# norabelrose/sparse-vae

Hardware: AMD Instinct MI355X
Metric: training tokens/sec + ELBO match vs CPU ref, 512-tok seq, 1/2/4/8 MI355X (higher is better)
Workload: dtype bf16; 1 GPU; c2: TransformerVAE 6L d512 heads 8 seq 512, batch 64/GPU, dense attention, dropout 0.1, fwd+bwd+allreduce+clip+RAdam; model=TransformerVAE-6L-d512, global_batch=64, seq_len=512, parallelism=dp1

## Files before the change

include/svae.h:

```cpp
#ifndef SVAE_H
#define SVAE_H
#include <stdint.h>
#ifdef __cplusplus
extern "C" {
#endif

typedef void* svae_stream_t;

enum svae_epi {
  SVAE_EPI_BF16 = 0,
  SVAE_EPI_F32 = 1,
  SVAE_EPI_F32_ACC = 2,
  SVAE_EPI_F32_ATOMIC = 3,
  SVAE_EPI_GELU = 4,
  SVAE_EPI_GELU_BWD = 5,
  SVAE_EPI_DROPOUT_RESID = 6,
  SVAE_EPI_ROTARY_BF16 = 7,
  SVAE_EPI_CE_STATS = 8,
  SVAE_EPI_CE_PROB = 9,
  SVAE_EPI_ROWSCALE_GATHER = 10
};

typedef struct svae_gemm_desc {
  const void* A;
// ... 15 lines not shown
  uint64_t seed;
  const float* rot_tab;
  int32_t rot_cols, rot_d, rot_seq;
  const int32_t* labels;
  float* label_logit;
  float* a_rowsum;
  const float* k_weight;
  const float* row_a;
  const float* row_b;
  const void* gather;
  int64_t ldg;
  float* delta;
  const float* delta_o32;
  int64_t ld_o32;
  int32_t delta_hd, delta_seq;
} svae_gemm_desc;

int svae_gemm(const svae_gemm_desc* d, svae_stream_t stream);

int svae_gemm_pair(const svae_gemm_desc* d0, const svae_gemm_desc* d1, svae_stream_t stream);

#define SVAE_GROUP_MAX 256
#define SVAE_GROUP_MAX_BLOCKS 1024
int64_t svae_gemm_group_table_bytes(int32_t n);
int svae_gemm_group(const svae_gemm_desc* d, int32_t n, int32_t max_blocks, void* table, void* table_host,
                    int64_t table_bytes, svae_stream_t stream);

int svae_resid_ln_fwd(const float* x, const void* y, int32_t y_dtype, int64_t ldy, float drop_p, uint64_t seed,
                      const float* zrows, int32_t zmod, const float* w, const float* b, float* xo, void* h, float* mean,
                      float* rstd, int32_t rows, int32_t D, svae_stream_t stream);
// ... 18 lines not shown
int svae_layernorm_bwd_multi(const void* const* dy, const float* x, const float* const* w, const float* mean,
                             const float* rstd, const float* dres, float* dx, float* const* part, int32_t nblk,
                             int32_t n, int32_t rows, int32_t D, svae_stream_t stream);

int svae_colsum(const void* in, int32_t in_dtype, int32_t rows, int32_t cols, int64_t ld, float* out,
                int32_t accumulate, svae_stream_t stream);

#define SVAE_COLSUM_MAX 8
typedef struct svae_colsum_seg {
  const float* in;
  float* out;
  int64_t ld;
  int32_t rows, cols;
} svae_colsum_seg;
int svae_colsum_multi(const svae_colsum_seg* segs, int32_t n, svae_stream_t stream);

typedef struct svae_attn_desc {
  const void* q; const void* k; const void* v; void* o;
  int64_t sq, sk, sv, so, bq, bk, bv, bo;
  const uint8_t* key_pad;
  float* lse;
  int32_t B, H, Lq, Lk, hd, causal;
  float scale;
  const void* dout; int64_t sdo, bdo;
  float* delta;
  float* dq;
  int64_t bdq;
  void* dk; void* dv;
  int64_t sdk, sdv, bdk, bdv;
  const float* rot_tab;
// ... 153 lines not shown
```

sparse-vae_amd/csrc/gemm.hip:

```cpp
#include "common.h"
#include "../../include/svae.h"
#include <stdlib.h>
#include <string.h>
#include <algorithm>
#include <vector>

using namespace svae;

namespace {

constexpr int BM = 128, BN = 128, BK = 64;
constexpr int TILE_BYTES = BM * BK * 2;

struct GP {
  const bf16* A; const bf16* B;
  long long lda, ldb, sA, sB;
  int M, N, K, splits, kchunk, tiles_n, tiles_m;
  void* C; long long ldc, sC;
  const float* bias;
  const float* resid; long long ldr;
  void* aux; long long ldaux;
  float alpha, drop_p;
  unsigned long long seed;
  const float* rot_tab; int rot_cols, rot_d, rot_seq;
  const int* labels; float* label_logit;
  float* a_rowsum;
  const float* k_weight;
  const float* row_a; const float* row_b;
  const bf16* gather; long long ldg;
  int epi;
  int tn2, tm2;
  int group;
  int total3;
  int relaxed;
  int dma_stagger;
  long long slab;
  float* delta; const float* delta_o32; long long ld_o32; int delta_hd, delta_seq;
};

__device__ __forceinline__ int kc_off(int row, int c) { return row * 128 + ((c ^ ((row >> 1) & 7)) << 4); }
__device__ __forceinline__ int mn_off(int k, int u) {
  const int s = (k & 3) | (((k >> 3) & 1) << 2);
  return k * 256 + ((u ^ (s << 2)) << 3);
}

template <bool TRANS>
__device__ __forceinline__ void load_tile(const bf16* __restrict__ g, long long ld, int row0, int nrows, int k0,
                                          int kend, u32x4 (&r)[4], int tid) {
  const bf16* base = TRANS ? g + (long long)k0 * ld + row0 : g + (long long)row0 * ld + k0;
  const __amdgpu_buffer_rsrc_t rsrc = __builtin_amdgcn_make_buffer_rsrc((void*)base, 0, 0x7FFFFFF0, 0x00020000);
#pragma unroll
  for (int i = 0; i < 4; ++i) {
// ... 491 lines not shown
            cs[row * 128 + cs_swz(row, col)] = p.alpha * acc[i][j][r];
          }
    }
    __syncthreads();
    epilogue_half<EPI>(p, cs, m0, n0, bn, h * 64, cofs, tid);
    __syncthreads();
  }
}

constexpr int G3_T = 256 * 64 * 2;
constexpr int G3_STAGE = 2 * G3_T;
constexpr int G3_EPI_BF16_DELTA = 65;
constexpr int G3_EPI_ACC_KW = 64;
constexpr int G3_EPI_F32_KW = 66;
constexpr int G3_EPI_SLAB = 67;

struct G3Src {
  int off[4];
};

__device__ __forceinline__ void g3_piece_k(int piece, int lane, int& r, int& c) {
  r = piece * 8 + (lane >> 3);
  c = (lane & 7) ^ ((r >> 1) & 7);
}
__device__ __forceinline__ void g3_piece_mn(int piece, int lane, int& kr, int& col) {
  const int half = piece >> 4;
  kr = (piece & 15) * 4 + (lane >> 4);
  const int sk = (kr & 3) | (((kr >> 3) & 1) << 2);
  col = half * 128 + (((lane & 15) ^ (sk << 1)) * 8);
}
// ... 481 lines not shown
#ifndef SVAE_KW_FORM
#define SVAE_KW_FORM 0
#endif
#ifndef SVAE_KW_PRE
#define SVAE_KW_PRE 1
#endif

template <int EPI>
constexpr int g3_epi_vmem_ops() {
  switch (EPI) {
    case SVAE_EPI_BF16:
    case G3_EPI_BF16_DELTA:
    case SVAE_EPI_ROTARY_BF16:
    case SVAE_EPI_CE_STATS:
    case SVAE_EPI_ROWSCALE_GATHER:
    case SVAE_EPI_GELU_BWD:
      return 8 * 2;
    case SVAE_EPI_CE_PROB:
      return 8 * 2 + 1;
    case SVAE_EPI_GELU:
      return 8 * 2 * 2;
    case SVAE_EPI_F32:
    case SVAE_EPI_F32_ACC:
    case SVAE_EPI_DROPOUT_RESID:
    case G3_EPI_ACC_KW:
    case G3_EPI_F32_KW:
    case G3_EPI_SLAB:
      return 8 * 4;
    default:
      return 0;
  }
}

template <bool AT, bool BT, int EPI>
__device__ __forceinline__ void gemm256_run(const GP& p, int blk, int nwg, bool remap = true) {
  static_assert(g3_epi_vmem_ops<EPI>() >= G3_EPI_STORES, "the relaxed first wait would not cover the prefetch DMA");
  constexpr bool IS_KW = EPI == G3_EPI_ACC_KW || EPI == G3_EPI_F32_KW;
  constexpr int KW_FORM = IS_KW ? SVAE_KW_FORM : 0;
  constexpr int KW_SLOT = KW_FORM == 2 ? 1024 : 256;
  constexpr int KW_BYTES = KW_FORM ? 2 * 8 * KW_SLOT : 0;
  constexpr int RING_OFF = KW_FORM == 3 ? KW_BYTES : 0;
  constexpr int KW_OFF = KW_FORM == 3 ? 0 : 2 * G3_STAGE + 2048 + 8192;
  __shared__ __attribute__((aligned(16))) char smem[2 * G3_STAGE + 2048 + 8192 + KW_BYTES];
  char* ring = smem + RING_OFF;
  float* sbias = (float*)(ring + 2 * G3_STAGE);
  int* slabel = (int*)(ring + 2 * G3_STAGE + 1024);
  float* sstat = (float*)(ring + 2 * G3_STAGE + 2048);
  const int tid = threadIdx.x, lane = tid & 63;
  const int wave = __builtin_amdgcn_readfirstlane(tid >> 6);
  const int wr = wave >> 2, wc = wave & 3;
  int bid = blk;
  if (remap && nwg >= 16) {
    const int q = nwg / 8, r = nwg % 8, xcd = bid % 8, idx = bid / 8;
    bid = (xcd < r ? xcd * (q + 1) : r * (q + 1) + (xcd - r) * q) + idx;
  }
  int t3 = bid;
  if (t3 >= p.total3) return;
  G3Tile T = g3_tile(p, t3);
// ... 19 lines not shown
  bool relaxed = false;
  int ntile = 0;
  (void)ntile;
  while (true) {
    G3_STAMP(0);
    const int t3n = t3 + nwg;
    const bool has_next = t3n < p.total3;
    float rsum[4] = {0.f, 0.f, 0.f, 0.f};
    f32x4 acc[8][4];
#pragma unroll
    for (int i = 0; i < 8; ++i)
#pragma unroll
      for (int j = 0; j < 4; ++j) acc[i][j] = (f32x4){0.f, 0.f, 0.f, 0.f};

    const bool next_dma = has_next && g3_tile(p, t3n).nk > 0;
    for (int kt = 0; kt < T.nk; ++kt, ++g) {
      if (kt == 0 && relaxed) asm volatile("s_waitcnt vmcnt(%0)" ::"n"(G3_EPI_STORES) : "memory");
      else asm volatile("s_waitcnt vmcnt(0)" ::: "memory");
      __builtin_amdgcn_s_barrier();
      const char* la = ring + (g & 1) * G3_STAGE;
      const char* lb = la + G3_T;
      char* nxt = ring + ((g + 1) & 1) * G3_STAGE;
      const bool do_rs = AT && p.a_rowsum && T.bn < 2;
      const int ks0 = p.tn2 >= 2 ? T.bn : 0, ks1 = p.tn2 >= 2 ? T.bn + 1 : 2;
      const bool kw_pre = IS_KW && KW_FORM == 0 && SVAE_KW_PRE && do_rs;
      float kw1 = 0.f;
      if (kw_pre) {
        const int kk = T.kbeg + kt * 64 + lane_id_fresh();
        const int off = kk < T.kend ? kk * 4 : 0x7FFFFFF0;
        const u32x4 kwr = buffer_rsrc(p.k_weight, 0x7FFFFFF0u);
        asm volatile("s_nop 4\n\tbuffer_load_dword %0, %1, %2, 0 offen" : "=&v"(kw1) : "v"(off), "s"(kwr) : "memory");
      }
      const bool late = (!IS_KW || KW_FORM > 0 || kw_pre) && p.dma_stagger && wr == 1 && kt + 1 < T.nk;
      if (kt + 1 < T.nk) {
        if (!late) g3_issue<AT, BT>(p, T.A, T.B, sa, sb, T.m0, T.n0, T.kbeg + (kt + 1) * 64, T.kend, nxt, wave);
        kw_issue(T.kbeg + (kt + 1) * 64, T.kend, (g + 1) & 1);
      } else if (next_dma) {
        const G3Tile TN = g3_tile(p, t3n);
// ... 50 lines not shown
#pragma unroll
      for (int j = 0; j < 2; ++j)
#pragma unroll
        for (int ks = 0; ks < 2; ++ks) b1[j][ks] = g3_bfrag<BT>(lb, wc * 64 + 32 + j * 16, ks, lane);
#pragma unroll
      for (int ks = 0; ks < 2; ++ks)
#pragma unroll
        for (int i = 0; i < 4; ++i)
#pragma unroll
          for (int j = 0; j < 2; ++j) acc[i][j] = mfma16(b0[j][ks], a0[i][ks], acc[i][j]);
      if (late) {
        __builtin_amdgcn_sched_barrier(0);
        g3_issue<AT, BT>(p, T.A, T.B, sa, sb, T.m0, T.n0, T.kbeg + (kt + 1) * 64, T.kend, nxt, wave);
        __builtin_amdgcn_sched_barrier(0);
      }
      if constexpr (!AT) {
#pragma unroll
        for (int i = 0; i < 4; ++i)
#pragma unroll
          for (int ks = 0; ks < 2; ++ks) a1[i][ks] = g3_afrag<AT>(la, wr * 128 + 64 + i * 16, ks, lane);
      }
#pragma unroll
      for (int ks = 0; ks < 2; ++ks)
#pragma unroll
        for (int i = 0; i < 4; ++i)
#pragma unroll
          for (int j = 0; j < 2; ++j) acc[i][2 + j] = mfma16(b1[j][ks], a0[i][ks], acc[i][2 + j]);
      if constexpr (AT) {
        if (kw_pre) asm volatile("s_waitcnt vmcnt(8)" : "+v"(kw1) :: "memory");
        if (do_rs) {
// ... 11 lines not shown
        for (int i = 0; i < 4; ++i)
#pragma unroll
          for (int j = 0; j < 2; ++j) acc[4 + i][2 + j] = mfma16(b1[j][ks], a1[i][ks], acc[4 + i][2 + j]);
#pragma unroll
      for (int ks = 0; ks < 2; ++ks)
#pragma unroll
        for (int i = 0; i < 4; ++i)
#pragma unroll
          for (int j = 0; j < 2; ++j) acc[4 + i][j] = mfma16(b0[j][ks], a1[i][ks], acc[4 + i][j]);
      if constexpr (AT) {
        if (do_rs) {
          if (wc == 2) rowsum2(a1[0], a1[1]);
          else if (wc == 3) rowsum2(a1[2], a1[3]);
        }
      }
    }
    G3_STAMP(1);
    if (tid < 256) {
      const int n = T.n0 + tid, m = T.m0 + tid;
      sbias[tid] = (p.bias && n < p.N) ? p.bias[n] : 0.f;
      if (EPI == SVAE_EPI_CE_STATS || EPI == SVAE_EPI_CE_PROB || EPI == SVAE_EPI_ROWSCALE_GATHER)
        slabel[tid] = m < p.M ? p.labels[m] : 0;
      if (EPI == SVAE_EPI_CE_PROB) sstat[1024 + tid] = (m < p.M && p.labels[m] != 0) ? p.row_a[m] : INFINITY;
      if (EPI == SVAE_EPI_ROWSCALE_GATHER) sstat[1024 + tid] = m < p.M ? p.row_a[m] : 0.f;
      if (EPI == SVAE_EPI_ROWSCALE_GATHER) sstat[1280 + tid] = m < p.M ? p.row_b[m] : 0.f;
    }
    asm volatile("s_waitcnt lgkmcnt(0)" ::: "memory");
    __builtin_amdgcn_s_barrier();
    if constexpr (AT) {
      if (p.a_rowsum && T.bn < 2) {
#pragma unroll
        for (int h = 0; h < 2; ++h) {
          const float t = sum_x16_x32(rsum[h]);
          const int m = T.m0 + wr * 128 + (2 * wc + h) * 16 + (lane & 15);
          if ((lane >> 4) == 0 && m < p.M) atomicAdd(p.a_rowsum + m, t);
        }
      }
    }
    if constexpr (EPI == SVAE_EPI_BF16 || EPI == SVAE_EPI_GELU || EPI == SVAE_EPI_CE_STATS ||
                  EPI == SVAE_EPI_ROTARY_BF16 || EPI == SVAE_EPI_CE_PROB)
      g3_reg_epilogue<EPI>(p, acc, sbias, slabel, sstat, T.m0, T.n0, T.bn, T.batch, T.split, wr, wc, tid, lane);
    else if constexpr (EPI == SVAE_EPI_ROWSCALE_GATHER)
      g3_rowscale_gather_epilogue(p, acc, slabel, sstat + 1024, sstat + 1280, T.m0, T.n0, wr, wc, lane);
    else if constexpr (EPI == SVAE_EPI_F32 || EPI == SVAE_EPI_F32_ACC || EPI == SVAE_EPI_DROPOUT_RESID ||
                       EPI == SVAE_EPI_GELU_BWD || EPI == G3_EPI_BF16_DELTA)
      g3_reg_epilogue_ld<EPI>(p, acc, sbias, T.m0, T.n0, T.batch, T.split, wr, wc, lane);
    else if constexpr (EPI == G3_EPI_ACC_KW)
      g3_reg_epilogue_ld<SVAE_EPI_F32_ACC>(p, acc, sbias, T.m0, T.n0, T.batch, T.split, wr, wc, lane);
    else if constexpr (EPI == G3_EPI_F32_KW || EPI == G3_EPI_SLAB)
      g3_reg_epilogue_ld<G3_EPI_SLAB>(p, acc, sbias, T.m0, T.n0, T.batch, T.split, wr, wc, lane);
    else
      static_assert(EPI == G3_EPI_SLAB, "no gemm256 epilogue for this EPI");
    relaxed = p.relaxed && T.m0 + 256 <= p.M && T.n0 + 256 <= p.N;
    G3_STAMP(2);
    ++ntile;
    if (!has_next) break;
    const bool prefetched = T.nk > 0;
// ... 167 lines not shown
__global__ __launch_bounds__(256) void slab_reduce_kernel(SlabRed r) { slab_reduce_range(r, blockIdx.x, gridDim.x); }
__global__ __launch_bounds__(256) void slab_reduce2_kernel(SlabRed r0, SlabRed r1, int nb0) {
  if ((int)blockIdx.x < nb0) slab_reduce_range(r0, blockIdx.x, nb0);
  else slab_reduce_range(r1, blockIdx.x - nb0, (int)gridDim.x - nb0);
}
struct alignas(16) SlabRedSlot {
  SlabRed r;
};
__global__ __launch_bounds__(256) void slab_reduce_list_kernel(const SlabRedSlot* __restrict__ list, int n) {
  for (int e = 0; e < n; ++e) {
    const SlabRed r = load_uniform(&list[e].r);
    slab_reduce_range(r, blockIdx.x, gridDim.x);
  }
}

}

static SlabRed slab_red(const svae_gemm_desc* d) {
  return SlabRed{(const float*)d->aux, (float*)d->C, d->M, d->N, (long long)d->ldc, d->splits};
}
static long long slab_blocks(const svae_gemm_desc* d) {
  return std::min(4096LL, ((long long)d->M * (d->N / 4) + 255) / 256);
}
static int launch_slab_reduce(const svae_gemm_desc* d, hipStream_t s) {
  hipLaunchKernelGGL(slab_reduce_kernel, dim3((unsigned)slab_blocks(d)), dim3(256), 0, s, slab_red(d));
  SVAE_LAUNCH_CHECK();
  return SVAE_OK;
}

static int validate_desc(const svae_gemm_desc* d) {
// ... 10 lines not shown
  if (d->epi == SVAE_EPI_CE_PROB && !d->aux) return SVAE_EINVAL;
  if (d->epi == SVAE_EPI_ROWSCALE_GATHER && (!d->row_b || !d->gather || d->ldg % 8 || ((uintptr_t)d->gather & 15)))
    return SVAE_EINVAL;
  if (d->k_weight && (!d->a_rowsum || !d->a_t || (d->splits != 1 && !(d->epi == SVAE_EPI_F32_ATOMIC && d->aux))))
    return SVAE_EINVAL;
  if (d->epi == SVAE_EPI_ROTARY_BF16 && (!d->rot_tab || d->rot_d <= 0 || d->rot_seq <= 0)) return SVAE_EINVAL;
  if ((d->epi == SVAE_EPI_GELU || d->epi == SVAE_EPI_GELU_BWD || d->epi == SVAE_EPI_CE_STATS) && !d->aux)
    return SVAE_EINVAL;
  if (d->epi == SVAE_EPI_DROPOUT_RESID && !d->resid) return SVAE_EINVAL;
  if ((d->epi == SVAE_EPI_DROPOUT_RESID || d->epi == SVAE_EPI_F32) && d->aux &&
      (d->batch != 1 || d->ldaux % 8 || ((uintptr_t)d->aux & 15)))
    return SVAE_EINVAL;
  if (d->epi == SVAE_EPI_CE_STATS && (!d->labels || !d->label_logit || d->splits != 1)) return SVAE_EINVAL;
  if (d->splits > 1 && d->epi != SVAE_EPI_F32_ATOMIC) return SVAE_EINVAL;
  if (d->a_rowsum && !d->a_t) return SVAE_EINVAL;
  if (d->N % 4 || d->ldc % 8 || ((uintptr_t)d->C & 15) || (d->resid && (d->ldr % 4 || ((uintptr_t)d->resid & 15))))
    return SVAE_EINVAL;
  if ((d->epi == SVAE_EPI_GELU || d->epi == SVAE_EPI_GELU_BWD) && (d->ldaux % 8 || ((uintptr_t)d->aux & 15)))
    return SVAE_EINVAL;
  if (d->epi == SVAE_EPI_ROTARY_BF16 && (d->rot_d % 4 || d->rot_cols % 4)) return SVAE_EINVAL;

  return SVAE_OK;
}

static void fill_gp(const svae_gemm_desc* d, GP& p) {
  p.A = (const bf16*)d->A; p.B = (const bf16*)d->B;
  p.lda = d->lda; p.ldb = d->ldb; p.sA = d->batch_stride_a; p.sB = d->batch_stride_b;
  p.M = d->M; p.N = d->N; p.K = d->K; p.splits = d->splits;
  int kchunk = (d->K + d->splits - 1) / d->splits;
  kchunk = (kchunk + BK - 1) / BK * BK;
// ... 3 lines not shown
  p.C = d->C; p.ldc = d->ldc; p.sC = d->batch_stride_c;
  p.bias = d->bias; p.resid = d->resid; p.ldr = d->ldr;
  p.aux = d->aux; p.ldaux = d->ldaux;
  p.alpha = d->alpha; p.drop_p = d->drop_p; p.seed = d->seed;
  p.rot_tab = d->rot_tab; p.rot_cols = d->rot_cols; p.rot_d = d->rot_d; p.rot_seq = d->rot_seq;
  p.labels = d->labels; p.label_logit = d->label_logit;
  p.a_rowsum = d->a_rowsum;
  p.k_weight = d->k_weight;
  p.row_a = d->row_a; p.row_b = d->row_b;
  p.gather = (const bf16*)d->gather; p.ldg = d->ldg;
  p.epi = d->epi;
  p.slab = 0;
  p.dma_stagger = 0;
  p.delta = d->delta; p.delta_o32 = d->delta_o32; p.ld_o32 = d->ld_o32;
  p.delta_hd = d->delta_hd; p.delta_seq = d->delta_seq;
}

__global__ __launch_bounds__(256) void gemm_delta_kernel(const bf16* __restrict__ C, long long ldc,
                                                         const float* __restrict__ o32, long long ldo, int M, int H,
                                                         int hd, int seq, float* __restrict__ delta) {
  const int gw = blockIdx.x * 4 + (threadIdx.x >> 6), lane = threadIdx.x & 63;
  if (gw >= M * H) return;
  const int m = gw / H, h = gw - m * H;
  float s = 0.f;
  for (int c = lane * 4; c < hd; c += 256) {
    const bf16x4 a = *(const bf16x4*)(C + (long long)m * ldc + h * hd + c);
    const f32x4 o = *(const f32x4*)(o32 + (long long)m * ldo + h * hd + c);
#pragma unroll
    for (int e = 0; e < 4; ++e) s = fmaf((float)a[e], o[e], s);
  }
// ... 125 lines not shown
      case G3_EPI_SLAB:
        hipLaunchKernelGGL((gemm256_kernel<true, true, G3_EPI_SLAB>), grid3, dim3(512), 0, s, p);
        break;
      case G3_EPI_F32_KW:
        if (!d->b_t) return SVAE_EINVAL;
        hipLaunchKernelGGL((gemm256_kernel<true, true, G3_EPI_F32_KW>), grid3, dim3(512), 0, s, p);
        break;
      case SVAE_EPI_CE_PROB:
        hipLaunchKernelGGL((gemm256_kernel<false, false, SVAE_EPI_CE_PROB>), grid3, dim3(512), 0, s, p);
        break;
      case G3_EPI_BF16_DELTA:
        if (d->b_t) hipLaunchKernelGGL((gemm256_kernel<false, true, G3_EPI_BF16_DELTA>), grid3, dim3(512), 0, s, p);
        else hipLaunchKernelGGL((gemm256_kernel<false, false, G3_EPI_BF16_DELTA>), grid3, dim3(512), 0, s, p);
        break;
      case SVAE_EPI_ROWSCALE_GATHER:
        if (d->b_t) hipLaunchKernelGGL((gemm256_kernel<false, true, SVAE_EPI_ROWSCALE_GATHER>), grid3, dim3(512), 0, s, p);
        else hipLaunchKernelGGL((gemm256_kernel<false, false, SVAE_EPI_ROWSCALE_GATHER>), grid3, dim3(512), 0, s, p);
        break;
      default: return SVAE_EINVAL;
    }
#undef SVAE_GEMM3_CASE
    SVAE_LAUNCH_CHECK();
    return slab ? launch_slab_reduce(d, s) : SVAE_OK;
  }
  if (impl == 2) {
    int kchunk2 = (d->K + d->splits - 1) / d->splits;
    p.kchunk = (kchunk2 + BK2 - 1) / BK2 * BK2;
#define SVAE_GEMM2_CASE(E)                                                                             \
  case E:                                                                                              \
    if (lay == 0) hipLaunchKernelGGL((gemm_glds_kernel<false, false, E>), grid, dim3(256), 0, s, p);    \
    else if (lay == 1) hipLaunchKernelGGL((gemm_glds_kernel<false, true, E>), grid, dim3(256), 0, s, p); \
// ... 246 lines not shown
```

sparse-vae_amd/sparse_vae/_native.py:

```python
import ctypes
import os

import torch

_HERE = os.path.dirname(os.path.abspath(__file__))
LIB_PATH = os.environ.get('SVAE_LIB') or os.path.join(_HERE, 'libsvae.so')

c_void_p, c_int32, c_int64, c_float, c_uint64 = (ctypes.c_void_p, ctypes.c_int32, ctypes.c_int64,
                                                  ctypes.c_float, ctypes.c_uint64)
c_fptr = ctypes.c_void_p

EPI_BF16, EPI_F32, EPI_F32_ACC, EPI_F32_ATOMIC, EPI_GELU, EPI_GELU_BWD, EPI_DROPOUT_RESID, \
    EPI_ROTARY_BF16, EPI_CE_STATS, EPI_CE_PROB, EPI_ROWSCALE_GATHER = range(11)

LATENT_L2, LATENT_COSINE, LATENT_KL = range(3)
LATENT_METRICS = {'l2': LATENT_L2, 'cosine': LATENT_COSINE, 'kl': LATENT_KL}
LATENT_MAX_BLOCKS = 1024


class GemmDesc(ctypes.Structure):
    _fields_ = [
        ('A', c_void_p), ('B', c_void_p),
        ('lda', c_int64), ('ldb', c_int64), ('batch_stride_a', c_int64), ('batch_stride_b', c_int64),
        ('M', c_int32), ('N', c_int32), ('K', c_int32),
        ('batch', c_int32), ('splits', c_int32),
        ('a_t', c_int32), ('b_t', c_int32),
        ('epi', c_int32),
        ('C', c_void_p),
        ('ldc', c_int64), ('batch_stride_c', c_int64),
        ('bias', c_void_p), ('resid', c_void_p), ('ldr', c_int64),
        ('aux', c_void_p), ('ldaux', c_int64),
        ('alpha', c_float), ('drop_p', c_float), ('seed', c_uint64),
        ('rot_tab', c_void_p), ('rot_cols', c_int32), ('rot_d', c_int32), ('rot_seq', c_int32),
        ('labels', c_void_p), ('label_logit', c_void_p),
        ('a_rowsum', c_void_p),
        ('k_weight', c_void_p), ('row_a', c_void_p), ('row_b', c_void_p), ('gather', c_void_p), ('ldg', c_int64),
        ('delta', c_void_p), ('delta_o32', c_void_p), ('ld_o32', c_int64), ('delta_hd', c_int32), ('delta_seq', c_int32),
    ]


class AttnDesc(ctypes.Structure):
    _fields_ = [
        ('q', c_void_p), ('k', c_void_p), ('v', c_void_p), ('o', c_void_p),
        ('sq', c_int64), ('sk', c_int64), ('sv', c_int64), ('so', c_int64),
        ('bq', c_int64), ('bk', c_int64), ('bv', c_int64), ('bo', c_int64),
        ('key_pad', c_void_p), ('lse', c_void_p),
        ('B', c_int32), ('H', c_int32), ('Lq', c_int32), ('Lk', c_int32), ('hd', c_int32), ('causal', c_int32),
        ('scale', c_float),
        ('dout', c_void_p), ('sdo', c_int64), ('bdo', c_int64),
        ('delta', c_void_p), ('dq', c_void_p), ('bdq', c_int64),
        ('dk', c_void_p), ('dv', c_void_p),
        ('sdk', c_int64), ('sdv', c_int64), ('bdk', c_int64), ('bdv', c_int64),
# ... 34 lines not shown
    'svae_gemm_group': [ctypes.POINTER(GemmDesc), c_int32, c_int32, c_void_p, c_void_p, c_int64, c_void_p],
    'svae_resid_ln_fwd': [c_void_p, c_void_p, c_int32, c_int64, c_float, c_uint64, c_void_p, c_int32, c_void_p,
                          c_void_p, c_void_p, c_void_p, c_void_p, c_void_p, c_int32, c_int32, c_void_p],
    'svae_layernorm_fwd': [c_void_p, c_int32, c_void_p, c_void_p, c_void_p, c_void_p, c_void_p, c_int32, c_int32,
                           c_void_p],
    'svae_layernorm_bwd': [c_void_p, c_void_p, c_int32, c_void_p, c_void_p, c_void_p, c_void_p, c_void_p, c_void_p,
                           c_void_p, c_int32, c_int32, c_int32, c_int32, c_void_p],
    'svae_layernorm_bwd_drop': [c_void_p, c_void_p, c_int32, c_void_p, c_void_p, c_void_p, c_void_p, c_void_p,
                                c_void_p, c_void_p, c_int32, c_int32, c_int32, c_int32, c_float, c_uint64, c_int32,
                                c_void_p, c_void_p, c_void_p],
    'svae_layernorm_bwd_gelu': [c_void_p, c_void_p, c_int32, c_void_p, c_void_p, c_void_p, c_void_p, c_void_p,
                                c_void_p, c_int32, c_int32, c_int32, c_void_p],
    'svae_layernorm_nblk': [c_int32],
    'svae_colsum': [c_void_p, c_int32, c_int32, c_int32, c_int64, c_void_p, c_int32, c_void_p],
    'svae_colsum_multi': [c_void_p, c_int32, c_void_p],
    'svae_attn_fwd': [ctypes.POINTER(AttnDesc), c_void_p],
    'svae_attn_bwd': [ctypes.POINTER(AttnDesc), c_void_p],
    'svae_attn_dq_part_elems': [c_int32, c_int32, c_int32, c_int32, c_int32],
    'svae_attn_dq_part_elems_w': [c_int32, c_int32, c_int32, c_int32, c_int32, c_int32],
    'svae_attn_fwd_ws_elems': [c_int32, c_int32, c_int32, c_int32, c_int32, c_int32, c_int32],
    'svae_transpose_blocks': [c_void_p, c_void_p, c_void_p, c_int32, c_int32, c_void_p],
    'svae_dq_finalize': [c_void_p, c_void_p, c_int64, c_int32, c_int32, c_void_p, c_int32, c_void_p],
    'svae_embedding_fwd': [c_void_p, c_void_p, c_void_p, c_void_p, c_int32, c_int32, c_void_p],
    'svae_embedding_fwd_dual': [c_void_p, c_void_p, c_void_p, c_void_p, c_int32, c_int32, c_void_p],
    'svae_embedding_bwd': [c_void_p, c_void_p, c_void_p, c_int32, c_int32, c_void_p],
    'svae_reparam_kl_fwd': [c_void_p, c_void_p, c_uint64, c_void_p, c_void_p, c_void_p, c_void_p, c_void_p,
                            c_void_p, c_int32, c_int32, c_void_p],
    'svae_reparam_kl_bwd': [c_void_p, c_void_p, c_void_p, c_void_p, c_void_p, c_void_p, c_int32, c_int32, c_void_p],
    'svae_ce_finalize': [c_void_p, c_int32, c_void_p, c_void_p, c_int32, c_int32, c_int32, c_int32, c_void_p,
                         c_void_p, c_void_p, c_void_p, c_void_p, c_void_p],
# ... 95 lines not shown
```

sparse-vae_amd/sparse_vae/engine.py:

```python
import math
import os
from collections import OrderedDict

import torch

from . import kernels as K
from ._native import COLSUM_MAX, GROUP_MAX, LN_MULTI_MAX, ZPROJ_MAX
from ._native import EPI_BF16, EPI_F32, EPI_F32_ACC, EPI_GELU, EPI_GELU_BWD, EPI_DROPOUT_RESID, \
    EPI_ROTARY_BF16, EPI_CE_STATS, EPI_F32_ATOMIC, EPI_CE_PROB, EPI_ROWSCALE_GATHER

bf16, f32 = torch.bfloat16, torch.float32
ALIGN = 64
CE_CHUNK_NUMEL = 2 ** 30


def _attn_entries(pre, d, learned):
    out = []
    if learned:
        out.append((pre + 'learned_queries', (1, learned, d)))
        names = ['k_linear', 'v_linear']
    else:
        names = ['q_linear', 'k_linear', 'v_linear']
    out += [(pre + n + '.weight', (d, d)) for n in names]
    out += [(pre + n + '.bias', (d,)) for n in names]
# ... 185 lines not shown
        self.saved = None
        self.probe = None
        self.head_mode = os.environ.get('SVAE_HEAD', 'prob')
        assert self.head_mode in ('prob', 'logits'), self.head_mode
        self.dw_pair = os.environ.get('SVAE_DW_PAIR', '1') != '0'
        self.dw_group = os.environ.get('SVAE_DW_GROUP', '1') != '0'
        self._dw_jobs = []
        self._dwq = None
        self._dw_names = False
        self._dwg_states, self._dwg_sched = [], {}
        self.fuse_ln = os.environ.get('SVAE_FUSE_LN', '0') != '0'
        self.delta_fused = os.environ.get('SVAE_DELTA_FUSED', '0') != '0'
        self.o32_mode = os.environ.get('SVAE_ATTN_O32', '0') != '0'
        self.resid_bf16 = os.environ.get('SVAE_RESID_BF16', '1') != '0'
        self.head_g2 = os.environ.get('SVAE_HEAD_G2', '1') != '0'
        self.ln_gelu = os.environ.get('SVAE_LN_GELU', '1') != '0'
        self.small_fused = os.environ.get('SVAE_SMALL_FUSED', '1') != '0'
        self.zp_batch = os.environ.get('SVAE_ZPROJ_BATCH', '1') != '0'
        self.zf_batch = os.environ.get('SVAE_ZPROJ_FWD_BATCH', '1') != '0'
        self._zp_pending, self._zp_ctx = [], None
        self.cs_batch = os.environ.get('SVAE_COLSUM_BATCH', '1') != '0'
        self._cs_pending = []
        self.ncu = (torch.cuda.get_device_properties(flat.device).multi_processor_count
                    if flat.device.type == 'cuda' else 256)
        self.side = None
        if flat.device.type == 'cuda' and os.environ.get('SVAE_DW_STREAM', '0') != '0':
            self.side = torch.cuda.Stream(device=flat.device)

    def rot(self, L, window=0):
        need = max(L, self.hp.num_latents)
# ... 719 lines not shown
            gs[0:1].copy_(gl)
            gs[1:2].copy_(gl * kl_weight)

        logits = sv['logits']
        dhh = ws.get('b.dhh', (T, d))
        nch, clen = sv['nchunks'], sv['chunk_len']
        if sv['head'] == 'prob':
            hh = sv['hh']
            hh_r = ws.get('b.hh_r', (T, d))
            r_t = ws.get('b.ce_r', (T,), f32)
            q_t = ws.get('b.ce_q', (T,), f32)
            dbias = P.g('output_layer.3.bias')
            K.ce_prob_bwd_prep(hh, sv['lse'], sv['coff'], sv['chunk_w'], sv['labels'], gs[0:1], T, L, nch, clen, d, hh_r,
                               r_t, q_t, dbias)
            s = self._head_dw_splits(V, d)
            if s == 1:
                K.gemm(logits, hh_r, P.g('input_layer.0.weight'), V, d, T, a_t=True, b_t=True, lda=V, ldb=d, ldc=d,
                       epi=EPI_F32_ACC, a_rowsum=dbias, k_weight=r_t)
            else:
                slab = ws.get('b.head_dw_slab', (s * V * d,), f32)
                K.gemm(logits, hh_r, P.g('input_layer.0.weight'), V, d, T, a_t=True, b_t=True, lda=V, ldb=d, ldc=d,
                       epi=EPI_F32_ATOMIC, splits=s, aux=slab, a_rowsum=dbias, k_weight=r_t)
            W = P.w('input_layer.0.weight')
            K.gemm(logits, P.wT('input_layer.0.weight', V, d), dhh, T, d, V, epi=EPI_ROWSCALE_GATHER,
                   labels=sv['labels'], row_a=r_t, row_b=q_t, gather=W, ldg=d)
            sv['ce_q'] = q_t
        else:
            K.ce_grad(logits, V, sv['lse'], sv['chunk_w'], sv['labels'], gs[0:1], T, V, L, nch, clen)
            self._dw(logits, sv['hh'], 'input_layer.0.weight', T, V, d, bias='output_layer.3.bias', on_side=False)
            K.gemm(logits, P.wT('input_layer.0.weight', V, d), dhh, T, d, V, epi=EPI_BF16)
        dpre0 = ws.get('b.dpre0', (T, d))
        if self.ln_gelu:
            self._ln_bwd('output_layer.2', dhh, sv['ln_h'], T, None, None, dx_bf=dpre0, gelu=sv['gp0'])
        else:
            dh0 = ws.get('b.dh0', (T, d), f32)
            self._ln_bwd('output_layer.2', dhh, sv['ln_h'], T, None, dh0)
            K.gelu_bwd(dh0, sv['gp0'], dpre0, T * d)
        self._dw(dpre0, sv['xf'], 'output_layer.0.weight', T, d, d, bias='output_layer.0.bias')
        dx = ws.get('b.dx_dec', (T, d), f32)
        top = sv['dec_layers'][-1]
# ... 87 lines not shown
```

sparse-vae_amd/sparse_vae/kernels.py:

```python
import ctypes
import os

import torch

from . import _native as N
from ._native import lib, check, ptr, stream

bf16, f32 = torch.bfloat16, torch.float32

_gemm_desc = N.GemmDesc()


def _dev(*ts):
    for t in ts:
        if t is not None and not t.is_cuda:
            raise RuntimeError('libsvae kernels need device tensors (no CPU fallback)')


def gemm(A, B, C, M, N_, K, *, a_t=False, b_t=False, lda=None, ldb=None, ldc=None, epi=N.EPI_BF16, bias=None,
         resid=None, ldr=0, aux=None, ldaux=0, alpha=1.0, splits=1, drop_p=0.0, seed=0, rot=None, rot_cols=0,
         rot_d=0, rot_seq=0, labels=None, label_logit=None, batch=1, sA=0, sB=0, sC=0, a_rowsum=None, k_weight=None,
         row_a=None, row_b=None, gather=None, ldg=0, delta=None, delta_o32=None, ld_o32=0, delta_hd=0, delta_seq=0):
    d = _fill_desc(_gemm_desc, A, B, C, M, N_, K, a_t=a_t, b_t=b_t, lda=lda, ldb=ldb, ldc=ldc, epi=epi, bias=bias,
                   resid=resid, ldr=ldr, aux=aux, ldaux=ldaux, alpha=alpha, splits=splits, drop_p=drop_p, seed=seed,
                   rot=rot, rot_cols=rot_cols, rot_d=rot_d, rot_seq=rot_seq, labels=labels, label_logit=label_logit,
                   batch=batch, sA=sA, sB=sB, sC=sC, a_rowsum=a_rowsum, k_weight=k_weight, row_a=row_a, row_b=row_b,
                   gather=gather, ldg=ldg)
    if delta is not None:
        _dev(delta, delta_o32)
        assert delta.dtype == f32 and delta_o32.dtype == f32 and delta.numel() >= M * (N_ // delta_hd)
    d.delta, d.delta_o32, d.ld_o32 = ptr(delta), ptr(delta_o32), ld_o32
    d.delta_hd, d.delta_seq = delta_hd, delta_seq
    check(lib.svae_gemm(ctypes.byref(d), stream()), 'svae_gemm')


def _fill_desc(d, A, B, C, M, N_, K, *, a_t=False, b_t=False, lda=None, ldb=None, ldc=None, epi=N.EPI_BF16,
               bias=None, resid=None, ldr=0, aux=None, ldaux=0, alpha=1.0, splits=1, drop_p=0.0, seed=0, rot=None,
               rot_cols=0, rot_d=0, rot_seq=0, labels=None, label_logit=None, batch=1, sA=0, sB=0, sC=0,
               a_rowsum=None, k_weight=None, row_a=None, row_b=None, gather=None, ldg=0):
    _dev(A, B, C)
    assert A.dtype == bf16 and B.dtype == bf16
    d.A, d.B = A.data_ptr(), B.data_ptr()
    d.lda = lda if lda is not None else (M if a_t else K)
    d.ldb = ldb if ldb is not None else (N_ if b_t else K)
    d.batch_stride_a, d.batch_stride_b = sA, sB
    d.M, d.N, d.K = M, N_, K
    d.batch, d.splits = batch, splits
# ... 7 lines not shown
    d.ldr = ldr
    d.aux = ptr(aux)
    d.ldaux = ldaux
    d.alpha = alpha
    d.drop_p = drop_p
    d.seed = seed & 0xFFFFFFFFFFFFFFFF
    d.rot_tab = ptr(rot)
    d.rot_cols, d.rot_d, d.rot_seq = rot_cols, rot_d, rot_seq
    d.labels = ptr(labels)
    d.label_logit = ptr(label_logit)
    d.a_rowsum = ptr(a_rowsum)
    d.k_weight = ptr(k_weight)
    d.row_a, d.row_b = ptr(row_a), ptr(row_b)
    d.gather, d.ldg = ptr(gather), ldg
    d.delta, d.delta_o32, d.ld_o32, d.delta_hd, d.delta_seq = None, None, 0, 0, 0
    return d


_pair_desc = (N.GemmDesc(), N.GemmDesc())


def gemm_pair(g0, g1):
    d0 = _fill_desc(_pair_desc[0], *g0[0], **g0[1])
    d1 = _fill_desc(_pair_desc[1], *g1[0], **g1[1])
    check(lib.svae_gemm_pair(ctypes.byref(d0), ctypes.byref(d1), stream()), 'svae_gemm_pair')


def auto_splits(M, N_, K, target=512):
    t256 = -(-M // 256) * -(-N_ // 256)
    if t256 >= 192:
# ... 236 lines not shown


def colsum_multi(segs):
    assert 0 < len(segs) <= N.COLSUM_MAX
    for i, (inp, rows, cols, ld, out) in enumerate(segs):
        _dev(inp, out)
        assert inp.dtype == f32 and out.dtype == f32
        _colsum_segs[i].inp, _colsum_segs[i].out = inp.data_ptr(), out.data_ptr()
        _colsum_segs[i].ld, _colsum_segs[i].rows, _colsum_segs[i].cols = ld, rows, cols
    check(lib.svae_colsum_multi(ctypes.addressof(_colsum_segs), len(segs), stream()), 'svae_colsum_multi')


def colsum(inp, rows, cols, ld, out, accumulate=True):
    check(lib.svae_colsum(inp.data_ptr(), 0 if inp.dtype == f32 else 1, rows, cols, ld, out.data_ptr(),
                          int(accumulate), stream()), 'svae_colsum')


_attn_desc = N.AttnDesc()


def attention(q, k, v, o, lse, *, B, H, Lq, Lk, hd, sq, sk, sv, so, bq, bk, bv, bo, key_pad=None, causal=False,
              window=0, scale=None, backward=False, dout=None, sdo=0, bdo=0, delta=None, dq=None, bdq=0, dk=None, dv=None,
              sdk=0, sdv=0, bdk=0, bdv=0, rot=None, rot_d=0, o32=None, so32=0, bo32=0, dq_part=None, dq_bf=None,
              ldq_bf=0, delta_ready=False, o_lo=None, so_lo=0, bo_lo=0):
    d = _attn_desc
    d.q, d.k, d.v, d.o = q.data_ptr(), k.data_ptr(), v.data_ptr(), o.data_ptr()
    d.sq, d.sk, d.sv, d.so, d.bq, d.bk, d.bv, d.bo = sq, sk, sv, so, bq, bk, bv, bo
    d.key_pad = ptr(key_pad)
    d.lse = lse.data_ptr()
    d.B, d.H, d.Lq, d.Lk, d.hd, d.causal = B, H, Lq, Lk, hd, int(causal)
# ... 388 lines not shown
```

Before: 2.740 million tokens/s.

## Compute head bias gradient column sums inside the rowscale-gather GEMM

The output-head bias gradient (a row-weighted column sum of the logits gradient) moves out of the head weight-gradient GEMM, where it was a k_weight rowsum. It is now computed inside the ROWSCALE_GATHER dX GEMM. A new epilogue variant splits row_a into three bf16 pieces and runs an extra MFMA per K-tile on the A tile already staged in LDS, producing per-256-row partial sums in a slab. A small kernel then reduces that slab into dbias. The aim is to take rowsum work off the weight-gradient GEMM's critical path, at the cost of extra LDS, MFMAs and stores in the dX GEMM plus one extra launch.

```diff
diff --git a/include/svae.h b/include/svae.h
--- a/include/svae.h
+++ b/include/svae.h
@@ -53,6 +53,7 @@
   const float* delta_o32;
   int64_t ld_o32;
   int32_t delta_hd, delta_seq;
+  float* a_colsum;
 } svae_gemm_desc;
 
 int svae_gemm(const svae_gemm_desc* d, svae_stream_t stream);
@@ -101,6 +102,8 @@
   int32_t rows, cols;
 } svae_colsum_seg;
 int svae_colsum_multi(const svae_colsum_seg* segs, int32_t n, svae_stream_t stream);
+
+int svae_colsum_slab(const float* slab, int32_t rows, int32_t cols, float* out, svae_stream_t stream);
 
 typedef struct svae_attn_desc {
   const void* q; const void* k; const void* v; void* o;
diff --git a/sparse-vae_amd/csrc/gemm.hip b/sparse-vae_amd/csrc/gemm.hip
--- a/sparse-vae_amd/csrc/gemm.hip
+++ b/sparse-vae_amd/csrc/gemm.hip
@@ -36,6 +36,7 @@
   int dma_stagger;
   long long slab;
   float* delta; const float* delta_o32; long long ld_o32; int delta_hd, delta_seq;
+  float* a_colsum;
 };
 
 __device__ __forceinline__ int kc_off(int row, int c) { return row * 128 + ((c ^ ((row >> 1) & 7)) << 4); }
@@ -557,6 +558,8 @@
 constexpr int G3_EPI_ACC_KW = 64;
 constexpr int G3_EPI_F32_KW = 66;
 constexpr int G3_EPI_SLAB = 67;
+constexpr int G3_EPI_RSG_COLSUM = 68;
+constexpr int G3_CS_BYTES = 4 * 256 * 2 + 2 * 8 * 256;
 
 struct G3Src {
   int off[4];
@@ -1068,6 +1071,7 @@
     case SVAE_EPI_ROTARY_BF16:
     case SVAE_EPI_CE_STATS:
     case SVAE_EPI_ROWSCALE_GATHER:
+    case G3_EPI_RSG_COLSUM:
     case SVAE_EPI_GELU_BWD:
       return 8 * 2;
     case SVAE_EPI_CE_PROB:
@@ -1095,7 +1099,12 @@
   constexpr int KW_BYTES = KW_FORM ? 2 * 8 * KW_SLOT : 0;
   constexpr int RING_OFF = KW_FORM == 3 ? KW_BYTES : 0;
   constexpr int KW_OFF = KW_FORM == 3 ? 0 : 2 * G3_STAGE + 2048 + 8192;
-  __shared__ __attribute__((aligned(16))) char smem[2 * G3_STAGE + 2048 + 8192 + KW_BYTES];
+  constexpr bool IS_CS = EPI == G3_EPI_RSG_COLSUM;
+  constexpr bool IS_RSG = EPI == SVAE_EPI_ROWSCALE_GATHER || IS_CS;
+  static_assert(!IS_CS || !AT, "a_colsum reads K-contiguous A fragments");
+  __shared__ __attribute__((aligned(16))) char smem[2 * G3_STAGE + 2048 + 8192 + KW_BYTES + (IS_CS ? G3_CS_BYTES : 0)];
+  bf16* scw = (bf16*)(smem + 2 * G3_STAGE + 2048 + 8192);
+  float* scs = (float*)(scw + 4 * 256);
   char* ring = smem + RING_OFF;
   float* sbias = (float*)(ring + 2 * G3_STAGE);
   int* slabel = (int*)(ring + 2 * G3_STAGE + 1024);
@@ -1145,6 +1154,48 @@
       for (int j = 0; j < 4; ++j) acc[i][j] = (f32x4){0.f, 0.f, 0.f, 0.f};
 
     const bool next_dma = has_next && g3_tile(p, t3n).nk > 0;
+    int cs_phase = 0, cs_pend = -1, cs_buf = 0;
+    if constexpr (IS_CS) {
+      if (tid < 256) {
+        const float w = T.m0 + tid < p.M ? p.row_a[T.m0 + tid] : 0.f;
+        const bf16 hi = f2bf(w);
+        const float r1 = w - bf2f(hi);
+        const bf16 mid = f2bf(r1);
+        scw[tid] = hi;
+        scw[256 + tid] = mid;
+        scw[512 + tid] = f2bf(r1 - bf2f(mid));
+        scw[768 + tid] = f2bf(0.f);
+      }
+    }
+    auto cs_flush = [&](int k0, int buf) {
+      const int lane = lane_id_fresh();
+      const float* src = scs + buf * 512 + lane;
+      float t = src[0];
+#pragma unroll
+      for (int w = 1; w < 8; ++w) t += src[w * 64];
+      if (k0 + lane < p.K) p.a_colsum[(long long)(T.m0 >> 8) * p.K + k0 + lane] = t;
+    };
+    auto colsum2 = [&](const char* la) {
+      const int lane = lane_id_fresh();
+      const int g8 = 8 * (lane >> 4), li = lane & 15, q = li >> 2, pp = lane & 3;
+      const int rb = wr * 128 + wc * 32;
+      const bf16x8 wf = *(const bf16x8*)(scw + min(li, 3) * 256 + rb + g8);
+      const int m = rb + g8 + q;
+      f32x4 cacc[4];
+#pragma unroll
+      for (int nt = 0; nt < 4; ++nt) {
+        const int c = 2 * nt + (pp >> 1);
+        const short4v lo = lds_read_tr(la + m * 128 + ((c ^ ((m >> 1) & 7)) << 4) + (pp & 1) * 8);
+        const short4v hi = lds_read_tr(la + (m + 4) * 128 + ((c ^ (((m + 4) >> 1) & 7)) << 4) + (pp & 1) * 8);
+        cacc[nt] = mfma16(wf, cat44(lo, hi), (f32x4){0.f, 0.f, 0.f, 0.f});
+      }
+      if (lane < 16) {
+        float* dst = scs + (cs_buf * 8 + wave) * 64 + lane;
+#pragma unroll
+        for (int nt = 0; nt < 4; ++nt) dst[16 * nt] = (cacc[nt][0] + cacc[nt][1]) + cacc[nt][2];
+      }
+      asm volatile("s_waitcnt lgkmcnt(0)" ::: "memory");
+    };
     for (int kt = 0; kt < T.nk; ++kt, ++g) {
       if (kt == 0 && relaxed) asm volatile("s_waitcnt vmcnt(%0)" ::"n"(G3_EPI_STORES) : "memory");
       else asm volatile("s_waitcnt vmcnt(0)" ::: "memory");
@@ -1153,6 +1204,8 @@
       const char* lb = la + G3_T;
       char* nxt = ring + ((g + 1) & 1) * G3_STAGE;
       const bool do_rs = AT && p.a_rowsum && T.bn < 2;
+      const bool cs_on = IS_CS && cs_phase == __builtin_amdgcn_readfirstlane(T.bn);
+      if constexpr (IS_CS) cs_phase = __builtin_amdgcn_readfirstlane(cs_phase + 1 == p.tn2 ? 0 : cs_phase + 1);
       const int ks0 = p.tn2 >= 2 ? T.bn : 0, ks1 = p.tn2 >= 2 ? T.bn + 1 : 2;
       const bool kw_pre = IS_KW && KW_FORM == 0 && SVAE_KW_PRE && do_rs;
       float kw1 = 0.f;
@@ -1233,6 +1286,10 @@
         g3_issue<AT, BT>(p, T.A, T.B, sa, sb, T.m0, T.n0, T.kbeg + (kt + 1) * 64, T.kend, nxt, wave);
         __builtin_amdgcn_sched_barrier(0);
       }
+      if constexpr (IS_CS) {
+        if (cs_pend >= 0 && wave == (kt & 3)) cs_flush(cs_pend, cs_buf ^ 1);
+        cs_pend = -1;
+      }
       if constexpr (!AT) {
 #pragma unroll
         for (int i = 0; i < 4; ++i)
@@ -1274,19 +1331,29 @@
           else if (wc == 3) rowsum2(a1[2], a1[3]);
         }
       }
+      if constexpr (IS_CS) {
+        if (cs_on) {
+          colsum2(la);
+          cs_pend = T.kbeg + kt * 64;
+          cs_buf ^= 1;
+        }
+      }
     }
     G3_STAMP(1);
     if (tid < 256) {
       const int n = T.n0 + tid, m = T.m0 + tid;
       sbias[tid] = (p.bias && n < p.N) ? p.bias[n] : 0.f;
-      if (EPI == SVAE_EPI_CE_STATS || EPI == SVAE_EPI_CE_PROB || EPI == SVAE_EPI_ROWSCALE_GATHER)
+      if (EPI == SVAE_EPI_CE_STATS || EPI == SVAE_EPI_CE_PROB || IS_RSG)
         slabel[tid] = m < p.M ? p.labels[m] : 0;
       if (EPI == SVAE_EPI_CE_PROB) sstat[1024 + tid] = (m < p.M && p.labels[m] != 0) ? p.row_a[m] : INFINITY;
-      if (EPI == SVAE_EPI_ROWSCALE_GATHER) sstat[1024 + tid] = m < p.M ? p.row_a[m] : 0.f;
-      if (EPI == SVAE_EPI_ROWSCALE_GATHER) sstat[1280 + tid] = m < p.M ? p.row_b[m] : 0.f;
+      if (IS_RSG) sstat[1024 + tid] = m < p.M ? p.row_a[m] : 0.f;
+      if (IS_RSG) sstat[1280 + tid] = m < p.M ? p.row_b[m] : 0.f;
     }
     asm volatile("s_waitcnt lgkmcnt(0)" ::: "memory");
     __builtin_amdgcn_s_barrier();
+    if constexpr (IS_CS) {
+      if (cs_pend >= 0 && wave == 0) cs_flush(cs_pend, cs_buf ^ 1);
+    }
     if constexpr (AT) {
       if (p.a_rowsum && T.bn < 2) {
 #pragma unroll
@@ -1300,7 +1367,7 @@
     if constexpr (EPI == SVAE_EPI_BF16 || EPI == SVAE_EPI_GELU || EPI == SVAE_EPI_CE_STATS ||
                   EPI == SVAE_EPI_ROTARY_BF16 || EPI == SVAE_EPI_CE_PROB)
       g3_reg_epilogue<EPI>(p, acc, sbias, slabel, sstat, T.m0, T.n0, T.bn, T.batch, T.split, wr, wc, tid, lane);
-    else if constexpr (EPI == SVAE_EPI_ROWSCALE_GATHER)
+    else if constexpr (IS_RSG)
       g3_rowscale_gather_epilogue(p, acc, slabel, sstat + 1024, sstat + 1280, T.m0, T.n0, wr, wc, lane);
     else if constexpr (EPI == SVAE_EPI_F32 || EPI == SVAE_EPI_F32_ACC || EPI == SVAE_EPI_DROPOUT_RESID ||
                        EPI == SVAE_EPI_GELU_BWD || EPI == G3_EPI_BF16_DELTA)
@@ -1498,6 +1565,34 @@
   }
 }
 
+__global__ __launch_bounds__(256) void colsum_slab_kernel(const float* __restrict__ slab, int rows, int cols,
+                                                          float* __restrict__ out) {
+  __shared__ f32x4 part[16][16];
+  const int cq = threadIdx.x & 15, rg = threadIdx.x >> 4;
+  const int c = blockIdx.x * 64 + cq * 4;
+  const int per = (rows + 15) / 16, r0 = rg * per, r1 = min(rows, r0 + per);
+  f32x4 acc = {0.f, 0.f, 0.f, 0.f};
+  if (c < cols)
+    for (int r = r0; r < r1; ++r) acc += *(const f32x4*)(slab + (long long)r * cols + c);
+  part[rg][cq] = acc;
+  __syncthreads();
+  if (rg == 0 && c < cols) {
+    f32x4 t = part[0][cq];
+#pragma unroll
+    for (int g = 1; g < 16; ++g) t += part[g][cq];
+    *(f32x4*)(out + c) += t;
+  }
+}
+
+}
+
+SVAE_EXPORT int svae_colsum_slab(const float* slab, int32_t rows, int32_t cols, float* out, svae_stream_t stream) {
+  if (!slab || !out || rows <= 0 || cols <= 0 || cols % 4 || (((uintptr_t)slab | (uintptr_t)out) & 15))
+    return SVAE_EINVAL;
+  hipLaunchKernelGGL(colsum_slab_kernel, dim3((unsigned)((cols + 63) / 64)), dim3(256), 0, (hipStream_t)stream, slab,
+                     (int)rows, (int)cols, out);
+  SVAE_LAUNCH_CHECK();
+  return SVAE_OK;
 }
 
 static SlabRed slab_red(const svae_gemm_desc* d) {
@@ -1538,6 +1633,9 @@
   if (d->epi == SVAE_EPI_CE_STATS && (!d->labels || !d->label_logit || d->splits != 1)) return SVAE_EINVAL;
   if (d->splits > 1 && d->epi != SVAE_EPI_F32_ATOMIC) return SVAE_EINVAL;
   if (d->a_rowsum && !d->a_t) return SVAE_EINVAL;
+  if (d->a_colsum && (d->epi != SVAE_EPI_ROWSCALE_GATHER || d->a_t || d->b_t || d->batch != 1 || d->splits != 1 ||
+                      ((uintptr_t)d->a_colsum & 15)))
+    return SVAE_EINVAL;
   if (d->N % 4 || d->ldc % 8 || ((uintptr_t)d->C & 15) || (d->resid && (d->ldr % 4 || ((uintptr_t)d->resid & 15))))
     return SVAE_EINVAL;
   if ((d->epi == SVAE_EPI_GELU || d->epi == SVAE_EPI_GELU_BWD) && (d->ldaux % 8 || ((uintptr_t)d->aux & 15)))
@@ -1571,6 +1669,7 @@
   p.dma_stagger = 0;
   p.delta = d->delta; p.delta_o32 = d->delta_o32; p.ld_o32 = d->ld_o32;
   p.delta_hd = d->delta_hd; p.delta_seq = d->delta_seq;
+  p.a_colsum = d->a_colsum;
 }
 
 __global__ __launch_bounds__(256) void gemm_delta_kernel(const bf16* __restrict__ C, long long ldc,
@@ -1726,7 +1825,8 @@
         else hipLaunchKernelGGL((gemm256_kernel<false, false, G3_EPI_BF16_DELTA>), grid3, dim3(512), 0, s, p);
         break;
       case SVAE_EPI_ROWSCALE_GATHER:
-        if (d->b_t) hipLaunchKernelGGL((gemm256_kernel<false, true, SVAE_EPI_ROWSCALE_GATHER>), grid3, dim3(512), 0, s, p);
+        if (d->a_colsum) hipLaunchKernelGGL((gemm256_kernel<false, false, G3_EPI_RSG_COLSUM>), grid3, dim3(512), 0, s, p);
+        else if (d->b_t) hipLaunchKernelGGL((gemm256_kernel<false, true, SVAE_EPI_ROWSCALE_GATHER>), grid3, dim3(512), 0, s, p);
         else hipLaunchKernelGGL((gemm256_kernel<false, false, SVAE_EPI_ROWSCALE_GATHER>), grid3, dim3(512), 0, s, p);
         break;
       default: return SVAE_EINVAL;
diff --git a/sparse-vae_amd/sparse_vae/_native.py b/sparse-vae_amd/sparse_vae/_native.py
--- a/sparse-vae_amd/sparse_vae/_native.py
+++ b/sparse-vae_amd/sparse_vae/_native.py
@@ -36,6 +36,7 @@
         ('a_rowsum', c_void_p),
         ('k_weight', c_void_p), ('row_a', c_void_p), ('row_b', c_void_p), ('gather', c_void_p), ('ldg', c_int64),
         ('delta', c_void_p), ('delta_o32', c_void_p), ('ld_o32', c_int64), ('delta_hd', c_int32), ('delta_seq', c_int32),
+        ('a_colsum', c_void_p),
     ]
 
 
@@ -100,6 +101,7 @@
     'svae_layernorm_nblk': [c_int32],
     'svae_colsum': [c_void_p, c_int32, c_int32, c_int32, c_int64, c_void_p, c_int32, c_void_p],
     'svae_colsum_multi': [c_void_p, c_int32, c_void_p],
+    'svae_colsum_slab': [c_void_p, c_int32, c_int32, c_void_p, c_void_p],
     'svae_attn_fwd': [ctypes.POINTER(AttnDesc), c_void_p],
     'svae_attn_bwd': [ctypes.POINTER(AttnDesc), c_void_p],
     'svae_attn_dq_part_elems': [c_int32, c_int32, c_int32, c_int32, c_int32],
diff --git a/sparse-vae_amd/sparse_vae/engine.py b/sparse-vae_amd/sparse_vae/engine.py
--- a/sparse-vae_amd/sparse_vae/engine.py
+++ b/sparse-vae_amd/sparse_vae/engine.py
@@ -223,6 +223,7 @@
         self.o32_mode = os.environ.get('SVAE_ATTN_O32', '0') != '0'
         self.resid_bf16 = os.environ.get('SVAE_RESID_BF16', '1') != '0'
         self.head_g2 = os.environ.get('SVAE_HEAD_G2', '1') != '0'
+        self.head_dbias_kw = os.environ.get('SVAE_HEAD_DBIAS', '') == 'kw'
         self.ln_gelu = os.environ.get('SVAE_LN_GELU', '1') != '0'
         self.small_fused = os.environ.get('SVAE_SMALL_FUSED', '1') != '0'
         self.zp_batch = os.environ.get('SVAE_ZPROJ_BATCH', '1') != '0'
@@ -972,16 +973,22 @@
             K.ce_prob_bwd_prep(hh, sv['lse'], sv['coff'], sv['chunk_w'], sv['labels'], gs[0:1], T, L, nch, clen, d, hh_r,
                                r_t, q_t, dbias)
             s = self._head_dw_splits(V, d)
+            kw = self.head_dbias_kw
             if s == 1:
                 K.gemm(logits, hh_r, P.g('input_layer.0.weight'), V, d, T, a_t=True, b_t=True, lda=V, ldb=d, ldc=d,
-                       epi=EPI_F32_ACC, a_rowsum=dbias, k_weight=r_t)
+                       epi=EPI_F32_ACC, a_rowsum=dbias if kw else None, k_weight=r_t if kw else None)
             else:
                 slab = ws.get('b.head_dw_slab', (s * V * d,), f32)
                 K.gemm(logits, hh_r, P.g('input_layer.0.weight'), V, d, T, a_t=True, b_t=True, lda=V, ldb=d, ldc=d,
-                       epi=EPI_F32_ATOMIC, splits=s, aux=slab, a_rowsum=dbias, k_weight=r_t)
+                       epi=EPI_F32_ATOMIC, splits=s, aux=slab, a_rowsum=dbias if kw else None,
+                       k_weight=r_t if kw else None)
             W = P.w('input_layer.0.weight')
+            nrt = -(-T // 256)
+            cs = None if kw else ws.get('b.head_dbias_slab', (nrt * V,), f32)
             K.gemm(logits, P.wT('input_layer.0.weight', V, d), dhh, T, d, V, epi=EPI_ROWSCALE_GATHER,
-                   labels=sv['labels'], row_a=r_t, row_b=q_t, gather=W, ldg=d)
+                   labels=sv['labels'], row_a=r_t, row_b=q_t, gather=W, ldg=d, a_colsum=cs)
+            if cs is not None:
+                K.colsum_slab(cs, nrt, V, dbias)
             sv['ce_q'] = q_t
         else:
             K.ce_grad(logits, V, sv['lse'], sv['chunk_w'], sv['labels'], gs[0:1], T, V, L, nch, clen)
diff --git a/sparse-vae_amd/sparse_vae/kernels.py b/sparse-vae_amd/sparse_vae/kernels.py
--- a/sparse-vae_amd/sparse_vae/kernels.py
+++ b/sparse-vae_amd/sparse_vae/kernels.py
@@ -20,7 +20,8 @@
 def gemm(A, B, C, M, N_, K, *, a_t=False, b_t=False, lda=None, ldb=None, ldc=None, epi=N.EPI_BF16, bias=None,
          resid=None, ldr=0, aux=None, ldaux=0, alpha=1.0, splits=1, drop_p=0.0, seed=0, rot=None, rot_cols=0,
          rot_d=0, rot_seq=0, labels=None, label_logit=None, batch=1, sA=0, sB=0, sC=0, a_rowsum=None, k_weight=None,
-         row_a=None, row_b=None, gather=None, ldg=0, delta=None, delta_o32=None, ld_o32=0, delta_hd=0, delta_seq=0):
+         row_a=None, row_b=None, gather=None, ldg=0, delta=None, delta_o32=None, ld_o32=0, delta_hd=0, delta_seq=0,
+         a_colsum=None):
     d = _fill_desc(_gemm_desc, A, B, C, M, N_, K, a_t=a_t, b_t=b_t, lda=lda, ldb=ldb, ldc=ldc, epi=epi, bias=bias,
                    resid=resid, ldr=ldr, aux=aux, ldaux=ldaux, alpha=alpha, splits=splits, drop_p=drop_p, seed=seed,
                    rot=rot, rot_cols=rot_cols, rot_d=rot_d, rot_seq=rot_seq, labels=labels, label_logit=label_logit,
@@ -31,6 +32,10 @@
         assert delta.dtype == f32 and delta_o32.dtype == f32 and delta.numel() >= M * (N_ // delta_hd)
     d.delta, d.delta_o32, d.ld_o32 = ptr(delta), ptr(delta_o32), ld_o32
     d.delta_hd, d.delta_seq = delta_hd, delta_seq
+    if a_colsum is not None:
+        _dev(a_colsum)
+        assert a_colsum.dtype == f32 and a_colsum.numel() >= -(-M // 256) * K
+    d.a_colsum = ptr(a_colsum)
     check(lib.svae_gemm(ctypes.byref(d), stream()), 'svae_gemm')
 
 
@@ -68,6 +73,7 @@
     d.row_a, d.row_b = ptr(row_a), ptr(row_b)
     d.gather, d.ldg = ptr(gather), ldg
     d.delta, d.delta_o32, d.ld_o32, d.delta_hd, d.delta_seq = None, None, 0, 0, 0
+    d.a_colsum = None
     return d
 
 
@@ -334,6 +340,12 @@
 def colsum(inp, rows, cols, ld, out, accumulate=True):
     check(lib.svae_colsum(inp.data_ptr(), 0 if inp.dtype == f32 else 1, rows, cols, ld, out.data_ptr(),
                           int(accumulate), stream()), 'svae_colsum')
+
+
+def colsum_slab(slab, rows, cols, out):
+    _dev(slab, out)
+    assert slab.dtype == f32 and out.dtype == f32 and slab.numel() >= rows * cols and out.numel() >= cols
+    check(lib.svae_colsum_slab(slab.data_ptr(), rows, cols, out.data_ptr(), stream()), 'svae_colsum_slab')
 
 
 _attn_desc = N.AttnDesc()
```

Result: no change. 2.765 million tokens/s, median of 6 (+0.9%).
